# imatge-upc/rsis

Measured on AMD Instinct MI355X. Metric: training images/sec at 256x256, T=10, batch=32 per GPU, higher is better.
Workload: dtype f32

## Files before the change

### include/rsis_hip.h

```cpp
#ifndef RSIS_HIP_H
#define RSIS_HIP_H
#include <stddef.h>
#ifdef __cplusplus
extern "C" {
#endif

#define RSIS_ABI_VERSION 2

#define RSIS_DTYPE_F32 0
#define RSIS_DTYPE_BF16 1
#define RSIS_DTYPE_BF16_BLK 2
#define RSIS_DTYPE_F32_WINO 3

int rsis_version(void);
const char* rsis_error_string(int code);
int rsis_conv_uses_wino(int ks, int stride, int pad, int Cin, int Cout, int nseg, int lstm_hid);

int rsis_set_deterministic(int on);
int rsis_get_deterministic(void);

int rsis_conv_uses_bf16(int ks, int stride, int pad, int Cout);
long rsis_conv_packed_bytes_fwd(int dtype, int Cout, int ks, int stride, int pad, int nseg, const int* Cseg);
long rsis_conv_packed_bytes_dgrad(int dtype, int Cout, int ks, int stride, int pad, int c_count);
int rsis_conv_pack_fwd(const float* W, void* Wp, int Cout, int Ctot, int ks, int stride, int pad, int nseg, const int* Cseg,
                       const int* Coff, int lstm_hid, int dtype, void* stream);
int rsis_conv_pack_dgrad(const float* W, void* Wd, int Cout, int Ctot, int ks, int stride, int pad, int nseg, const int* Cseg,
                         const int* Coff, int lstm_hid, int dtype, void* stream);

int rsis_conv2d_fwd(const float* const* src, const int* Csrc, int nsrc, int B, int H, int W, const void* Wp, int Cout,
                    int ks, int stride, int pad, const float* bias, const float* addend, float* out, int Ho, int Wo,
                    int tile, int dtype, void* stream);
int rsis_conv2d_fwd_bn_eval(const float* const* src, const int* Csrc, int nsrc, int B, int H, int W, const void* Wp, int Cout,
                            int ks, int stride, int pad, const float* bias, const float* addend, const float* gamma, const float* beta,
                            const float* running_mean, const float* running_var, float eps, int relu, float* out, int Ho, int Wo,
                            int tile, int dtype, void* stream);

int rsis_conv2d_dgrad(const float* dy, int B, int Cout, int Hy, int Wy, const void* Wd, int Cin_packed, int ks, int stride,
                      int pad, float* const* dx, const int* Cdx, int ndst, int Hx, int Wx, const float* addend, int tile,
                      int dtype, void* stream);

int rsis_conv2d_wgrad(const float* dy, const float* x, float* dW, int B, int Cs, int H, int W, int Cout, int Ho, int Wo,
                      int ks, int stride, int pad, int Ctot, int c_off, int lstm_hid, int dtype, void* stream);

typedef struct rsis_wgrad_job {
  const float* dy;
  const float* x;
  float* dW;
  int B, Cs, H, W, Cout, Ho, Wo, ks, stride, pad, Ctot, c_off, lstm_hid, dtype;
} rsis_wgrad_job;
int rsis_conv2d_wgrad_batch(const rsis_wgrad_job* jobs, int njobs, void* stream);

int rsis_bias_grad(const float* dy, float* db, int B, int C, int HW, int lstm_hid, void* stream);

int rsis_convlstm_fwd(const float* const* src, const int* Csrc, int nsrc, int B, int H, int W, const void* Wp,
                      const float* bias_packed, const float* addend, const float* c_prev, float* h_out, float* c_out,
                      float* act_out, int hid, int ks, int pad, int tile, int dtype, void* stream);

typedef struct rsis_lstm_job {
  const float* src[3];
  int Csrc[3];
  int nsrc, B, H, W;
  const void* Wp;
// ... 266 lines not shown
```

### rsis_amd/_lib.py

```python
import ctypes
import os

import torch

_HERE = os.path.dirname(os.path.abspath(__file__))
LIB_PATH = os.environ.get("RSIS_HIP_LIB") or os.path.join(_HERE, "lib", "librsis_hip.so")

_vp, _i, _l, _f = ctypes.c_void_p, ctypes.c_int, ctypes.c_long, ctypes.c_float
_ip = ctypes.POINTER(ctypes.c_int)
_vpp = ctypes.POINTER(ctypes.c_void_p)

class PackJob(ctypes.Structure):
    _fields_ = [("W", ctypes.c_void_p), ("out", ctypes.c_void_p), ("dgrad", ctypes.c_int), ("dtype", ctypes.c_int), ("Cout", ctypes.c_int),
                ("Ctot", ctypes.c_int), ("ks", ctypes.c_int), ("stride", ctypes.c_int), ("pad", ctypes.c_int),
                ("nseg", ctypes.c_int), ("Cseg", ctypes.c_int * 3), ("Coff", ctypes.c_int * 3), ("lstm_hid", ctypes.c_int),
                ("imode", ctypes.c_int), ("ldw", ctypes.c_int), ("krows", ctypes.c_int), ("block_begin", ctypes.c_int)]


class WgradJob(ctypes.Structure):
    _fields_ = [("dy", ctypes.c_void_p), ("x", ctypes.c_void_p), ("dW", ctypes.c_void_p)] + \
               [(k, ctypes.c_int) for k in ("B", "Cs", "H", "W", "Cout", "Ho", "Wo", "ks", "stride", "pad", "Ctot", "c_off", "lstm_hid", "dtype")]


class LstmJob(ctypes.Structure):
# ... 30 lines not shown


class BlkLstmBwdJob(ctypes.Structure):
    _fields_ = [(k, ctypes.c_void_p) for k in ("dh", "dh2", "dc_next", "act", "c_prev", "c", "da", "dc_prev")] + \
               [(k, ctypes.c_int) for k in ("B", "hid", "HW")]


SIGNATURES = {
    "rsis_version": (_i, []),
    "rsis_error_string": (ctypes.c_char_p, [_i]),
    "rsis_set_deterministic": (_i, [_i]),
    "rsis_get_deterministic": (_i, []),
    "rsis_conv_uses_bf16": (_i, [_i, _i, _i, _i]),
    "rsis_conv_uses_wino": (_i, [_i, _i, _i, _i, _i, _i, _i]),
    "rsis_conv_packed_bytes_fwd": (_l, [_i, _i, _i, _i, _i, _i, _ip]),
    "rsis_conv_packed_bytes_dgrad": (_l, [_i, _i, _i, _i, _i, _i]),
    "rsis_conv_pack_fwd": (_i, [_vp, _vp, _i, _i, _i, _i, _i, _i, _ip, _ip, _i, _i, _vp]),
    "rsis_conv_pack_dgrad": (_i, [_vp, _vp, _i, _i, _i, _i, _i, _i, _ip, _ip, _i, _i, _vp]),
    "rsis_conv_pack_job_fill": (_i, [ctypes.POINTER(PackJob)]),
    "rsis_conv_pack_batch": (_i, [_vp, _i, _i, _vp]),
    "rsis_conv2d_fwd": (_i, [_vpp, _ip, _i, _i, _i, _i, _vp, _i, _i, _i, _i, _vp, _vp, _vp, _i, _i, _i, _i, _vp]),
    "rsis_conv2d_fwd_bn_eval": (_i, [_vpp, _ip, _i, _i, _i, _i, _vp, _i, _i, _i, _i, _vp, _vp, _vp, _vp, _vp, _vp, _f, _i, _vp, _i, _i, _i, _i, _vp]),
    "rsis_conv2d_dgrad": (_i, [_vp, _i, _i, _i, _i, _vp, _i, _i, _i, _i, _vpp, _ip, _i, _i, _i, _vp, _i, _i, _vp]),
    "rsis_conv2d_wgrad": (_i, [_vp, _vp, _vp, _i, _i, _i, _i, _i, _i, _i, _i, _i, _i, _i, _i, _i, _i, _vp]),
    "rsis_conv2d_wgrad_batch": (_i, [ctypes.POINTER(WgradJob), _i, _vp]),
    "rsis_affine_nearest": (_i, [_vp, _vp, _vp, _i, _i, _i, _i, _i, _vp]),
    "rsis_targets_work_ints": (_l, [_i]),
    "rsis_targets_from_maps": (_i, [_vp, _vp, _i, _i, _i, _i, _vp, _vp, _vp, _vp, _vp, _vp]),
    "rsis_instance_maps_work_ints": (_l, [_i]),
    "rsis_instance_maps": (_i, [_vp, _vp, _i, _i, _i, _i, _vp, _vp, _vp, _vp]),
    "rsis_palette_to_ids": (_i, [_vp, _l, _vp, _i, _vp, _vp]),
    "rsis_idmap_rle_encode": (_i, [_vp, _i, _i, _vp, _i, _vp, _i, _vp, _vp]),
    "rsis_conv_out_wgrad": (_i, [_vp, _vp, _vp, _vp, _i, _i, _i, _i, _vp]),
    "rsis_conv_out_seq_fwd": (_i, [_vp, _vp, _vp, _vp, _i, _i, _i, _i, _i, _vp]),
    "rsis_conv_out_seq_dgrad": (_i, [_vp, _vp, _vp, _i, _i, _i, _i, _i, _vp]),
    "rsis_conv_out_seq_wgrad": (_i, [_vp, _vp, _vp, _vp, _i, _i, _i, _i, _i, _vp]),
    "rsis_sum_leading": (_i, [_vp, _vp, _i, _l, _vp]),
    "rsis_bias_grad": (_i, [_vp, _vp, _i, _i, _i, _i, _vp]),
    "rsis_convlstm_fwd": (_i, [_vpp, _ip, _i, _i, _i, _i, _vp, _vp, _vp, _vp, _vp, _vp, _vp, _i, _i, _i, _i, _i, _vp]),
    "rsis_convlstm_fwd_batch": (_i, [ctypes.POINTER(LstmJob), _i, _vp]),
    "rsis_convlstm_bwd_gates": (_i, [_vp, _vp, _vp, _vp, _vp, _vp, _vp, _vp, _vp, _i, _i, _i, _vp]),
    "rsis_upsample_bilinear_ac_fwd": (_i, [_vp, _vp, _l, _i, _i, _i, _i, _vp]),
    "rsis_upsample_bilinear_ac_bwd": (_i, [_vp, _vp, _l, _i, _i, _i, _i, _vp]),
    "rsis_upsample_maxpool_bwd": (_i, [_vp, _vp, _vp, _vp, _l, _i, _i, _i, _i, _vp]),
    "rsis_global_maxpool_fwd": (_i, [_vp, _vp, _vp, _l, _i, _vp]),
    "rsis_global_maxpool_bwd": (_i, [_vp, _vp, _vp, _l, _i, _vp]),
# ... 129 lines not shown
```

### rsis_amd/csrc/api.hip

```cpp
#include "common.h"
#include "../../include/rsis_hip.h"
#include <stdlib.h>

int rsis_launch_conv_igemm(ConvArgs& a, int ks, bool dgrad, int epi, int force_tile, hipStream_t st);
int rsis_launch_conv_wgrad(WgradArgs& a, int ks, hipStream_t st);
int rsis_launch_conv3x3_direct(ConvArgs& a, int epi, int force_variant, hipStream_t st);
int rsis_launch_conv_wino(const float* x, const void* U, const float* bias, const float* addend, float* y, int B, int C, int Cout, int H, int W,
                          hipStream_t st, int precise);
int rsis_launch_conv_wino_group(int n, const float* const* x, const void* const* U, float* const* y, float* const* y1, const int* B, const int* C,
                                const int* Cout, const int* C0, const int* H, const int* W, hipStream_t st);
int rsis_launch_convlstm_direct_group(ConvArgs* jobs, int n, const int* force_variant, hipStream_t st);
int rsis_launch_conv3x3_direct_group_plain(ConvArgs* jobs, int n, const int* force_variant, hipStream_t st);
int rsis_l_lstm_bwd_group(const void* const*, const int*, int, hipStream_t);
int rsis_launch_conv_bf16(ConvArgs& a, int ks, int epi, int force_variant, hipStream_t st);
int rsis_launch_conv_blk(ConvArgs& a, int ks, int variant, hipStream_t st);
int rsis_l_blk_from_nchw(const float*, void*, int, int, int, hipStream_t);
int rsis_l_blk_to_nchw(const void*, float*, int, int, int, hipStream_t);
long rsis_l_blk_bn_scratch(int);
int rsis_l_blk_bn_fwd(const void*, const void*, void*, double*, const float*, const float*, float*, float*, float*, float*, int, int, int, float,
                      float, int, int, hipStream_t);
int rsis_l_blk_bn_bwd(const void*, const void*, const void*, double*, const float*, const float*, const float*, const float*, void*, void*,
                      float*, float*, int, int, int, int, int, hipStream_t);
int rsis_l_blk_subsample(const void*, void*, long, int, int, int, int, int, hipStream_t);
int rsis_l_blk_upscatter(const void*, void*, long, int, int, int, int, int, hipStream_t);
// ... 468 lines not shown
      const int nq = (Cout + RSIS_CK - 1) / RSIS_CK;
      const long px_tiles = (long)B * rsis_cdiv(Hx, 8) * rsis_cdiv(Wx, Wx <= 8 ? 8 : 16);
      if (splitk_ok && !addend && nq >= 32 && px_tiles * rsis_cdiv(ctot, 64) < 160) {
        for (int i = 0; i < ndst; ++i)
          if (rsis_zero_async(dx[i], sizeof(float) * (size_t)B * Cdx[i] * Hx * Wx, (hipStream_t)stream) != RSIS_OK) return RSIS_ERR_LAUNCH;
        a.ksplit = 0;
      }
    }
    return rsis_launch_conv3x3_direct(a, 0, direct_variant(tile), (hipStream_t)stream);
  }
  if (use_direct_s2(ks, stride, pad) && ndst == 1 && Cdx[0] == Cin_packed && Hy == (Hx + 1) / 2 && Wy == (Wx + 1) / 2) {
    a.Ho = Hy; a.Wo = Wy; a.oH = Hx; a.oW = Wx;
    return rsis_launch_conv3x3_direct(a, 2, direct_variant(tile), (hipStream_t)stream);
  }
  if (ks == 1 && pad == 0 && stride > 1) {
    for (int i = 0; i < ndst && !inplace; ++i)
      if (rsis_zero_async(dx[i], sizeof(float) * (size_t)B * Cdx[i] * Hx * Wx, (hipStream_t)stream) != RSIS_OK) return RSIS_ERR_LAUNCH;
    a.Ho = Hy; a.Wo = Wy; a.stride = 1; a.sshift = 0; a.ostride = stride;
    return rsis_launch_conv_igemm(a, ks, false, 0, tile, (hipStream_t)stream);
  }
  return rsis_launch_conv_igemm(a, ks, true, 0, tile, (hipStream_t)stream);
}

static int wgrad_route(WgradArgs& a, int ks, int lstm_hid, int dtype) {
  if (dtype == RSIS_DTYPE_BF16_BLK) {
    a.blk = 1;
    return rsis_wgrad_bf16_supported(a, ks) ? 1 : -1;
  }
  if (use_direct(ks, a.stride, a.pad) && a.Cout == 1 && lstm_hid == 0 && rsis_c1_supported(a.Cs) && a.H == a.Ho && a.W == a.Wo && a.W % 4 == 0)
    return 0;
  if (dtype == RSIS_DTYPE_BF16 && rsis_wgrad_bf16_supported(a, ks)) return 1;
  static const bool tiled_ok = !(getenv("RSIS_WGRAD_TILED") && getenv("RSIS_WGRAD_TILED")[0] == '0');
  if (tiled_ok && rsis_wgrad_tiled_supported(a, ks)) return 2;
  return 3;
}
static int wgrad_fill(WgradArgs& a, const float* dy, const float* x, float* dW, int B, int Cs, int H, int W, int Cout, int Ho, int Wo,
                      int ks, int stride, int pad, int Ctot, int c_off, int lstm_hid) {
  if (!dy || !x || !dW || c_off < 0 || c_off + Cs > Ctot) return RSIS_ERR_ARG;
  a = WgradArgs{};
  a.dy = dy; a.x = x; a.dw = dW; a.B = B; a.Cs = Cs; a.H = H; a.W = W; a.Ho = Ho; a.Wo = Wo; a.Cout = Cout;
  a.stride = stride; a.pad = pad; a.ldo = Ctot * ks * ks; a.n_off = c_off * ks * ks; a.interleave_hid = lstm_hid;
  return RSIS_OK;
}
static int wgrad_launch_one(WgradArgs& a, int route, int ks, hipStream_t st) {
  switch (route) {
    case 0: return rsis_l_c1_wgrad(a.dy, a.x, a.dw + a.n_off, nullptr, a.B, a.Cs, a.H, a.W, 1, st);
// ... 636 lines not shown
```

### rsis_amd/csrc/common.h

```cpp
#pragma once
#include <hip/hip_runtime.h>
#include <stdint.h>

#define RSIS_OK 0
#define RSIS_ERR_ARG 1
#define RSIS_ERR_LAUNCH 2
#define RSIS_ERR_UNSUPPORTED 3

#define RSIS_KPAD 32
#define RSIS_CK 8
#define RSIS_CKB3 16
#define RSIS_CKB1 64
#define RSIS_LDW_ALIGN 128
#define RSIS_MAX_SRC 3

typedef float f32x16 __attribute__((ext_vector_type(16)));
typedef float f32x4 __attribute__((ext_vector_type(4)));

static inline int rsis_check_launch() {
  hipError_t e = hipGetLastError();
  return e == hipSuccess ? RSIS_OK : RSIS_ERR_LAUNCH;
}

int rsis_zero_async(void* p, size_t bytes, hipStream_t st);
// ... 40 lines not shown
  int Ho, Wo;
  int stride, pad, sshift;
  const float* wp;
  int ldw;
  int Cout;
  const float* bias;
  const float* addend;
  const float* ep_gamma; const float* ep_beta; const float* ep_mean; const float* ep_var;
  float ep_eps;
  int ep_relu, ep_round;
  float* dst[RSIS_MAX_SRC];
  int Cd[RSIS_MAX_SRC];
  int ndst;
  int n_co_tiles, n_px_tiles;
  int ostride, oH, oW;
  int ksplit;
  int hid;
  const float* c_prev;
  float* h_out;
  float* c_out;
  float* act_out;
  unsigned long long* side_key;
  int precise;
};

__device__ __forceinline__ unsigned long long rsis_side_key(float v, int idx) {
  unsigned u = __float_as_uint(v);
  u = (u & 0x80000000u) ? ~u : (u | 0x80000000u);
  return ((unsigned long long)u << 32) | (unsigned)(0x7FFFFFFF - idx);
}
__device__ __forceinline__ float rsis_side_value(unsigned long long k) {
  unsigned u = (unsigned)(k >> 32);
  u = (u & 0x80000000u) ? (u & 0x7FFFFFFFu) : ~u;
  return __uint_as_float(u);
}
__device__ __forceinline__ int rsis_side_index(unsigned long long k) { return 0x7FFFFFFF - (int)(unsigned)(k & 0xFFFFFFFFull); }
__device__ __forceinline__ unsigned long long rsis_key_max32(unsigned long long k) {
#pragma unroll
  for (int o = 16; o > 0; o >>= 1) {
    const unsigned long long t = __shfl_xor(k, o, 64);
    k = t > k ? t : k;
  }
  return k;
}

#define RSIS_SIDE_CHECK_TILES 192
// ... 87 lines not shown
```

### rsis_amd/csrc/conv_igemm.hip

```cpp
#include "common.h"
#include <type_traits>

enum { EPI_PLAIN = 0, EPI_LSTM = 1, EPI_BN = 2 };
#ifndef RSIS_GEMM_NST_DEFAULT
#define RSIS_GEMM_NST_DEFAULT 2
#endif

typedef const float __attribute__((address_space(1)))* gcf_t;
typedef const char __attribute__((address_space(1)))* gcc_t;
typedef float __attribute__((address_space(1)))* gf_t;
typedef const f32x4 __attribute__((address_space(1)))* gcf4_t;

typedef __attribute__((address_space(3))) void* lds_vp_t;
template <int BM, int BN, int BK, int WGM, int WGN, int KS, bool DGRAD, int EPI, bool V4, int NST = 2>
__global__ __launch_bounds__(256) void conv_igemm_kernel(const ConvArgs p) {
#if __HIP_DEVICE_COMPILE__
  constexpr int TM = BM / WGM / 32, TN = BN / WGN / 32;
  constexpr int KK = KS * KS;
  constexpr int B_ROWS = 256 / BN;
  constexpr int B_LOADS = BK / B_ROWS;
  constexpr int A_F4 = BK * BM / 4;
  constexpr int A_LOADS = (A_F4 + 255) / 256;
  static_assert(WGM * WGN == 4, "4 waves per block");
  static_assert(BN == 64 || BN == 128 || BN == 256, "BN");
  static_assert(RSIS_KPAD % BK == 0, "BK must divide the packed K padding");
  static_assert(!V4 || (KS == 1 && !DGRAD), "V4 is the 1x1 GEMM path");
// ... 216 lines not shown
    if constexpr (V4) {
      __builtin_amdgcn_s_waitcnt(0x0F70);
    } else {
      if (more) RSIS_STORE_TILE(cur ^ 1)
    }
    __syncthreads();
  }
  }
#undef RSIS_LOAD_TILE
#undef RSIS_STORE_TILE
#undef RSIS_DMA_TILE

  if constexpr (EPI == EPI_BN) {
    if (tid < BM) {
      const int row = co_t * BM + tid;
      float sc = 0.f, sh = 0.f;
      if (row < p.Cout) rsis_bn_affine(rsis_bn_eval_rstd(p.ep_var[row], p.ep_eps), p.ep_gamma[row], p.ep_beta[row], p.ep_mean[row], sc, sh);
      lds[tid] = sc; lds[BM + tid] = sh;
    }
    __syncthreads();
  }
  const int co_base = co_t * BM + wm * TM * 32;
  const gcf_t bias = (gcf_t)p.bias, addend = (gcf_t)p.addend;
  if (EPI == EPI_PLAIN || EPI == EPI_BN) {
    const gf_t d0 = (gf_t)p.dst[0], d1 = (gf_t)p.dst[1], d2 = (gf_t)p.dst[2];
    const int Cd0 = p.Cd[0], Cd1 = p.Cd[1], Cd2 = p.Cd[2], Cout = p.Cout;
    const int e1 = Cd0, e2 = Cd0 + Cd1;
    const int ostride = p.ostride, oHW = p.oH * p.oW;
#pragma unroll
    for (int j = 0; j < TN; ++j) {
      const int opx = px_t * BN + wn * TN * 32 + j * 32 + l31;
      if (opx >= Npx) continue;
      const int ob = opx / HoWo;
      int osp = opx - ob * HoWo;
      if (ostride > 1) { const int oho = osp / Wo; osp = (oho * ostride) * p.oW + (osp - oho * Wo) * ostride; }
      if (p.ndst == 1 && (size_t)p.B * Cout * oHW * 4 < (1ull << 31)) {
        const unsigned span = (unsigned)((size_t)p.B * Cout * oHW * 4);
        const __amdgpu_buffer_rsrc_t ro = __builtin_amdgcn_make_buffer_rsrc((void*)p.dst[0], 0, span, 0x00020000);
        const __amdgpu_buffer_rsrc_t ra = __builtin_amdgcn_make_buffer_rsrc((void*)(addend ? p.addend : p.dst[0]), 0, span, 0x00020000);
        const unsigned rowb = (unsigned)oHW * 4u;
#pragma unroll
        for (int i = 0; i < TM; ++i) {
          const int row0 = co_base + i * 32 + 4 * hi;
          const unsigned vo = (unsigned)((ob * Cout + row0) * oHW + osp) * 4u;
          const int rows_left = Cout - row0;
          float av[16];
          if (addend) {
#pragma unroll
            for (int r = 0; r < 16; ++r) {
              const int k = (r & 3) + 8 * (r >> 2);
              av[r] = __builtin_bit_cast(float, __builtin_amdgcn_raw_buffer_load_b32(ra, k < rows_left ? vo + k * rowb : 0x7FFFFFF0u, 0, 0));
            }
          }
          if constexpr (EPI == EPI_BN) {
            const float* tab = lds + wm * TM * 32 + i * 32 + 4 * hi;
#pragma unroll
            for (int g = 0; g < 4; ++g) {
              const f32x4 s4 = *reinterpret_cast<const f32x4*>(tab + 8 * g), h4 = *reinterpret_cast<const f32x4*>(tab + BM + 8 * g);
#pragma unroll
              for (int kk = 0; kk < 4; ++kk) {
                const int r = 4 * g + kk, k = kk + 8 * g;
                float v = acc[i][j][r];
                if (bias) v += k < rows_left ? bias[row0 + k] : 0.f;
                v = rsis_bn_apply(v, s4[kk], h4[kk], addend ? av[r] : 0.f, p.ep_relu);
                __builtin_amdgcn_raw_buffer_store_b32(__builtin_bit_cast(unsigned, v), ro, k < rows_left ? vo + k * rowb : 0x7FFFFFF0u, 0, 0);
              }
            }
            continue;
          }
#pragma unroll
          for (int r = 0; r < 16; ++r) {
            const int k = (r & 3) + 8 * (r >> 2);
            float v = acc[i][j][r];
            if (bias) v += k < rows_left ? bias[row0 + k] : 0.f;
            if (addend) v += av[r];
            __builtin_amdgcn_raw_buffer_store_b32(__builtin_bit_cast(unsigned, v), ro, k < rows_left ? vo + k * rowb : 0x7FFFFFF0u, 0, 0);
          }
        }
        continue;
      }
#pragma unroll
      for (int i = 0; i < TM; ++i) {
        if (addend) {
          float av[16];
#pragma unroll
          for (int r = 0; r < 16; ++r) {
            const int co = co_base + i * 32 + (r & 3) + 8 * (r >> 2) + 4 * hi;
            av[r] = co < Cout ? addend[((size_t)ob * Cd0 + co) * oHW + osp] : 0.f;
          }
#pragma unroll
          for (int r = 0; r < 16; ++r) {
            const int co = co_base + i * 32 + (r & 3) + 8 * (r >> 2) + 4 * hi;
            if (co < Cout) d0[((size_t)ob * Cd0 + co) * oHW + osp] = acc[i][j][r] + av[r] + (bias ? bias[co] : 0.f);
          }
          continue;
        }
#pragma unroll
        for (int r = 0; r < 16; ++r) {
// ... 38 lines not shown
          const size_t sidx = ((size_t)ob * hid + jh) * HoWo + osp;
          const float cp = c_prev ? c_prev[sidx] : 0.f;
          const float c = gf * cp + gi * gg;
          const float h = go * tanhf(c);
          c_out[sidx] = c;
          h_out[sidx] = h;
          if (act_out) {
            act_out[gidx] = gi; act_out[gidx + HoWo] = gf;
            act_out[gidx + 2 * (size_t)HoWo] = go; act_out[gidx + 3 * (size_t)HoWo] = gg;
          }
        }
      }
    }
  }
#endif
}

template <int BM, int BN, int BK, int WGM, int WGN, int KS, bool DGRAD, int EPI>
static int launch_cfg(ConvArgs& a, hipStream_t st) {
  const long Npx = (long)a.B * a.Ho * a.Wo;
  a.n_co_tiles = rsis_cdiv(a.Cout, BM);
  a.n_px_tiles = rsis_cdiv(Npx, BN);
  const int grid = a.n_co_tiles * 8 * rsis_cdiv(a.n_px_tiles, 8);
  if constexpr (KS == 1 && !DGRAD && (EPI == EPI_PLAIN || EPI == EPI_BN)) {
    if (a.stride == 1 && a.pad == 0 && a.nsrc == 1 && (a.H * a.W) % 4 == 0 && a.C[0] % BK == 0 &&
        (long)a.B * a.C[0] * a.H * a.W * 4 < (1L << 31)) {
      if constexpr (BM == 64 && BN == 64 && BK == 32 && EPI == EPI_PLAIN) {
        static const int nst = getenv("RSIS_GEMM_NST") ? atoi(getenv("RSIS_GEMM_NST")) : RSIS_GEMM_NST_DEFAULT;
        if (nst == 3) { hipLaunchKernelGGL((conv_igemm_kernel<BM, BN, BK, WGM, WGN, KS, DGRAD, EPI, true, 3>), dim3(grid), dim3(256), 0, st, a); return rsis_check_launch(); }
        if (nst == 4) { hipLaunchKernelGGL((conv_igemm_kernel<BM, BN, BK, WGM, WGN, KS, DGRAD, EPI, true, 4>), dim3(grid), dim3(256), 0, st, a); return rsis_check_launch(); }
      }
      hipLaunchKernelGGL((conv_igemm_kernel<BM, BN, BK, WGM, WGN, KS, DGRAD, EPI, true>), dim3(grid), dim3(256), 0, st, a);
      return rsis_check_launch();
    }
  }
  hipLaunchKernelGGL((conv_igemm_kernel<BM, BN, BK, WGM, WGN, KS, DGRAD, EPI, false>), dim3(grid), dim3(256), 0, st, a);
  return rsis_check_launch();
}

template <int KS, bool DGRAD, int EPI>
static int launch_ks(ConvArgs& a, hipStream_t st, int force_tile) {
  const long Npx = (long)a.B * a.Ho * a.Wo;
  int tile = force_tile;
  if (tile <= 0) {
    if (a.Cout <= 32) tile = (Npx >= 256L * 256) ? 1 : 2;
    else if (KS == 1) tile = 5;
    else if (a.Cout <= 64) tile = 3;
// ... 8 lines not shown
    case 2: return launch_cfg<32, 128, 16, 1, 4, KS, DGRAD, EPI>(a, st);
    case 3: return launch_cfg<64, 128, 16, 2, 2, KS, DGRAD, EPI>(a, st);
    case 4: return launch_cfg<128, 128, 16, 2, 2, KS, DGRAD, EPI>(a, st);
    case 5: return launch_cfg<64, 64, 16, 2, 2, KS, DGRAD, EPI>(a, st);
    case 6: return launch_cfg<128, 64, 16, 2, 2, KS, DGRAD, EPI>(a, st);
    case 11: return launch_cfg<32, 256, 32, 1, 4, KS, DGRAD, EPI>(a, st);
    case 12: return launch_cfg<32, 128, 32, 1, 4, KS, DGRAD, EPI>(a, st);
    case 13: return launch_cfg<64, 128, 32, 2, 2, KS, DGRAD, EPI>(a, st);
    case 14: return launch_cfg<128, 128, 32, 2, 2, KS, DGRAD, EPI>(a, st);
    case 15: return launch_cfg<64, 64, 32, 2, 2, KS, DGRAD, EPI>(a, st);
    case 16: return launch_cfg<128, 64, 32, 2, 2, KS, DGRAD, EPI>(a, st);
    default: return RSIS_ERR_ARG;
  }
}

int rsis_launch_conv_igemm(ConvArgs& a, int ks, bool dgrad, int epi, int force_tile, hipStream_t st) {
  if (a.nsrc < 0 || a.nsrc > RSIS_MAX_SRC) return RSIS_ERR_ARG;
  if (epi == EPI_LSTM) {
    if (dgrad) return RSIS_ERR_UNSUPPORTED;
    if (ks == 3) return launch_ks<3, false, EPI_LSTM>(a, st, force_tile);
    if (ks == 1) return launch_ks<1, false, EPI_LSTM>(a, st, force_tile);
    return RSIS_ERR_UNSUPPORTED;
  }
  if (a.ep_gamma) {
    if (dgrad || epi != EPI_PLAIN || a.ndst != 1 || a.Cout <= 32 || a.Cout % 4 != 0 || (size_t)a.B * a.Cout * a.oH * a.oW * 4 >= (1ull << 31))
      return RSIS_ERR_UNSUPPORTED;
    if (ks == 1) return launch_cfg<64, 64, 32, 2, 2, 1, false, EPI_BN>(a, st);
    if (ks == 7 && a.Cout <= 64) return launch_cfg<64, 128, 32, 2, 2, 7, false, EPI_BN>(a, st);
    return RSIS_ERR_UNSUPPORTED;
  }
  if (!dgrad) {
    if (ks == 1) return launch_ks<1, false, EPI_PLAIN>(a, st, force_tile);
    if (ks == 3) return launch_ks<3, false, EPI_PLAIN>(a, st, force_tile);
    if (ks == 7) return launch_ks<7, false, EPI_PLAIN>(a, st, force_tile);
  } else {
    if (ks == 1 && a.stride == 1 && a.pad == 0) return launch_ks<1, false, EPI_PLAIN>(a, st, force_tile);
    if (ks == 1) return launch_ks<1, true, EPI_PLAIN>(a, st, force_tile);
    if (ks == 3) return launch_ks<3, true, EPI_PLAIN>(a, st, force_tile);
    if (ks == 7) return launch_ks<7, true, EPI_PLAIN>(a, st, force_tile);
  }
  return RSIS_ERR_UNSUPPORTED;
}
```

### rsis_amd/ops.py

```python
import ctypes
import os
import weakref

import torch

from . import _lib
from ._lib import check, int_array, lib, ptr, ptr_array, require_cuda_f32, stream

_WEIGHT_EPOCH = [0]


FORCE_TILE = [0]


DIRECT_GRAD = [False]


def _direct_target(param):
    g = param.grad if DIRECT_GRAD[0] and param is not None else None
    return g if (g is not None and g.is_contiguous() and g.dtype == torch.float32 and g.is_cuda) else None


DTYPE_F32, DTYPE_BF16 = 0, 1
DTYPE_F32_WINO = 3
# ... 21 lines not shown
        return d
    return DTYPE_F32_WINO if (rule == "all" or (cin == cout and cin in rule)) else d

DTYPES = {"fp32": DTYPE_F32, "f32": DTYPE_F32, "float32": DTYPE_F32, "bf16": DTYPE_BF16, "bfloat16": DTYPE_BF16}


def set_dtype(module, dtype):
    d = DTYPES[dtype] if isinstance(dtype, str) else int(dtype)
    for m in module.modules():
        if hasattr(m, "_set_rsis_dtype"):
            m._set_rsis_dtype(d)
    return module


def set_deterministic(on=True):
    return bool(lib().rsis_set_deterministic(1 if on else 0))


def is_deterministic():
    return bool(lib().rsis_get_deterministic())


SUBSAMPLE_1X1 = [os.environ.get("RSIS_SUBSAMPLE_1X1", "1") != "0"]
_PACKS = weakref.WeakSet()
_BATCH = {"sig": None, "jobs": None, "n": 0, "blocks": 0}


def repack_all():
    L = lib()
    todo = []
    for p in list(_PACKS):
        w = p._refs[0]() if p._refs is not None else None
        if w is None or not w.is_cuda:
            continue
        b = p._refs[1]() if p._refs[1] is not None else None
        if p.wp is not None and p._key_f is not None:
            todo.append((p, w, b, p.wp, 0))
        if p.wd is not None and p._key_d is not None:
            todo.append((p, w, b, p.wd, 1))
    if not todo:
        return
    sig = tuple((id(p), w.data_ptr(), out.data_ptr(), d) for p, w, _b, out, d in todo)
    if _BATCH["sig"] != sig:
        jobs = (_lib.PackJob * len(todo))()
        blocks = 0
        for i, (p, w, _b, out, d) in enumerate(todo):
# ... 94 lines not shown
            L = lib()
            Cout, Ctot = w.shape[0], w.shape[1]
            nseg, segs, offs = self._seg_args()
            n = L.rsis_conv_packed_bytes_dgrad(self.dtype, Cout, self.ks, self.stride, self.pad, self.cin) // 4
            if self.wd is None or self.wd.numel() != n:
                self.wd = torch.zeros(n, dtype=torch.float32, device=w.device)
            check(L.rsis_conv_pack_dgrad(ptr(w.detach()), ptr(self.wd), Cout, Ctot, self.ks, self.stride, self.pad, nseg, segs, offs,
                                         self.lstm_hid, self.dtype, stream()), "rsis_conv_pack_dgrad")
            self._key_d = key
            if self._refs is None:
                self._refs = (weakref.ref(w), None)
            _PACKS.add(self)
        return self.wd


def _contig(t):
    return t if t.is_contiguous() else t.contiguous()


def _conv_out_size(n, ks, stride, pad):
    return (n + 2 * pad - ks) // stride + 1


def _dgrad_all(L, dy, wd, cin_packed, ks, stride, pad, srcs, Hx, Wx, addend=None, inplace=False, dtype=DTYPE_F32):
    B, Cout, Hy, Wy = dy.shape
    shapes = [tuple(s.shape) if torch.is_tensor(s) else tuple(s) for s in srcs]
    dxs = [addend] if inplace else [torch.empty(sh, dtype=torch.float32, device=dy.device) for sh in shapes]
    check(L.rsis_conv2d_dgrad(ptr(dy), B, Cout, Hy, Wy, ptr(wd), cin_packed, ks, stride, pad, ptr_array(dxs),
                              int_array([sh[1] for sh in shapes]), len(shapes), Hx, Wx, ptr(addend), FORCE_TILE[0], dtype, stream()),
          "rsis_conv2d_dgrad")
    return dxs


class GradSlot(object):

    def __init__(self):
        self.grad = None
        self.done = False

    def reset(self):
        self.grad, self.done = None, False

    def take(self):
        g, self.grad = self.grad, None
        self.done = True
        return g

    def park(self, g):
        if self.done or self.grad is not None or g is None:
            return False
        self.grad = g
        return True


class _GradTapFn(torch.autograd.Function):
    @staticmethod
    def forward(ctx, x, slot):
        ctx.slot = slot
        return x.view_as(x)

    @staticmethod
    def backward(ctx, g):
        if g is not None and ctx.slot.park(g if g.is_contiguous() else g.contiguous()):
            return None, None
        return g, None


def grad_tap(x, slot):
    if slot is None or not (torch.is_grad_enabled() and x.requires_grad):
        return x
    return _GradTapFn.apply(x, slot)


WGRAD_DEFER = [False]
# ... 43 lines not shown
        require_cuda_f32(weight, bias, *srcs)
        L = lib()
        B, _, H, W = srcs[0].shape
        Cout, ks = weight.shape[0], weight.shape[2]
        Ho, Wo = _conv_out_size(H, ks, stride, pad), _conv_out_size(W, ks, stride, pad)
        if pack.stride != stride or pack.pad != pad:
            raise _lib.RsisHipError("PackedConv was built for stride %d pad %d, used with %d/%d" % (pack.stride, pack.pad, stride, pad))
        wp = pack.fwd(weight)
        out = torch.empty((B, Cout, Ho, Wo), dtype=torch.float32, device=weight.device)
        ctx.in_shape = None
        if ks == 1 and stride > 1 and pad == 0 and nsrc == 1 and (SUBSAMPLE_1X1[0] or pack.dtype == DTYPE_BF16):
            ctx.in_shape = tuple(srcs[0].shape)
            sub = torch.empty((B, srcs[0].shape[1], Ho, Wo), dtype=torch.float32, device=weight.device)
            check(L.rsis_subsample2d(ptr(srcs[0]), ptr(sub), B * srcs[0].shape[1], H, W, stride, stream()), "rsis_subsample2d")
            srcs = [sub]
            H, W, stride_k = Ho, Wo, 1
        else:
            stride_k = stride
        tile = FORCE_TILE[0] + (100 if pack.training_call else 0)
        check(L.rsis_conv2d_fwd(ptr_array(srcs), int_array([s.shape[1] for s in srcs]), nsrc, B, H, W, ptr(wp), Cout, ks, stride_k,
                                pad, ptr(bias.detach() if bias is not None else None), None, ptr(out), Ho, Wo, tile, pack.dtype, stream()),
              "rsis_conv2d_fwd")
        ctx.pack, ctx.stride, ctx.pad, ctx.nsrc = pack, stride, pad, nsrc
        ctx.has_bias = bias is not None
        ctx.wparam, ctx.bparam = weight, bias
        ctx.save_for_backward(weight, *srcs)
        return out

    @staticmethod
    def backward(ctx, dy):
        weight = ctx.saved_tensors[0]
        srcs = list(ctx.saved_tensors[1:])
        dy = _contig(dy)
        L = lib()
        ks = weight.shape[2]
        nsrc = ctx.nsrc
        grads = [None] * (nsrc + 2)
        take, park = ctx.slot if isinstance(ctx.slot, tuple) else (ctx.slot, None)
        addend = take.take() if take is not None else None
        sub = ctx.in_shape is not None
        in_shapes = [ctx.in_shape] if sub else [tuple(t.shape) for t in srcs]
        if any(ctx.needs_input_grad[5:5 + nsrc]):
            wd = ctx.pack.dgrad(weight)
            inplace, extra = False, None
            if addend is not None:
                if nsrc != 1 or tuple(addend.shape) != in_shapes[0]:
                    raise _lib.RsisHipError("GradSlot: the parked gradient does not belong to this conv's input")
                if ctx.stride != 1:
                    if ks == 1 and ctx.pad == 0 and addend.is_contiguous():
                        inplace = True
                    else:
                        extra, addend = addend, None
            dxs = _dgrad_all(L, dy, wd, ctx.pack.cin, ks, ctx.stride, ctx.pad, in_shapes, in_shapes[0][2], in_shapes[0][3], addend,
                             inplace, dtype=ctx.pack.dtype)
            if extra is not None:
                dxs[0].add_(extra)
            for i in range(nsrc):
                if ctx.needs_input_grad[5 + i]:
                    grads[i] = dxs[i]
            if park is not None and nsrc == 1 and grads[0] is not None and park.park(grads[0]):
                grads[0] = None
        want_w = ctx.needs_input_grad[5 + nsrc]
        want_b = ctx.has_bias and ctx.needs_input_grad[6 + nsrc]
        if (want_w and want_b and weight.shape[0] == 1 and ks == 3 and ctx.stride == 1 and ctx.pad == 1 and nsrc == 1 and
                weight.shape[1] in (4, 8, 16) and srcs[0].shape[3] % 4 == 0):
            tw, tb = _direct_target(ctx.wparam), _direct_target(ctx.bparam)
            dW = tw if tw is not None else torch.zeros_like(weight)
            db = tb if tb is not None else torch.zeros(1, dtype=torch.float32, device=dy.device)
            x0 = srcs[0]
            check(L.rsis_conv_out_wgrad(ptr(dy), ptr(x0), ptr(dW), ptr(db), x0.shape[0], x0.shape[1], x0.shape[2], x0.shape[3], stream()),
                  "rsis_conv_out_wgrad")
            grads[nsrc] = None if tw is not None else dW
            grads[nsrc + 1] = None if tb is not None else db
            return (None, None, None, None, None) + tuple(grads)
        if want_w:
            tgt = _direct_target(ctx.wparam)
            dW = _wgrad_all(L, dy, srcs, tuple(weight.shape), ks, 1 if sub else ctx.stride, ctx.pad, 0, out=tgt, dtype=ctx.pack.dtype)
# ... 225 lines not shown
        x, y, gamma, mean, rstd = ctx.saved_tensors
        dy = _contig(dy)
        B, C, H, W = x.shape
        if not ctx.train:
            stats = torch.empty(2 * C, dtype=torch.float64, device=dy.device)
            dx = torch.empty_like(x)
            need_dres = ctx.has_res and ctx.relu
            dres = torch.empty_like(x) if need_dres else None
            dgamma = torch.empty(C, dtype=torch.float32, device=dy.device)
            dbeta = torch.empty_like(dgamma)
            fn, name = (lib().rsis_bn_bwd_eval_mask, "rsis_bn_bwd_eval_mask") if ctx.masked else (lib().rsis_bn_bwd_eval, "rsis_bn_bwd_eval")
            check(fn(ptr(dy), ptr(x), ptr(y), ptr(mean), ptr(rstd), ptr(gamma.detach()), ptr(stats), ptr(dx), ptr(dres),
                     ptr(dgamma), ptr(dbeta), B, C, H * W, float(ctx.eps), int(ctx.relu), stream()), name)
            if ctx.has_res and not need_dres:
                dres = dy
            return dx, dres, dgamma, dbeta, None, None, None, None, None, None, None, None, None
        flags = int(ctx.relu)
        if ctx.arena is not None:
            stats, flags = ctx.arena[1], flags | 2
        else:
            stats = torch.empty(2 * C, dtype=torch.float64, device=dy.device)
        dx = torch.empty_like(x)
        need_dres = ctx.has_res and ctx.relu
        dres = torch.empty_like(x) if need_dres else None
        tg, tb = _direct_target(ctx.gparam), _direct_target(ctx.bparam)
        direct = tg is not None and tb is not None
        if direct:
            dgamma, dbeta, flags = tg, tb, flags | 4
        else:
            dgamma = torch.empty(C, dtype=torch.float32, device=dy.device)
            dbeta = torch.empty_like(dgamma)
        fn, name = (lib().rsis_bn_bwd_mask, "rsis_bn_bwd_mask") if ctx.masked else (lib().rsis_bn_bwd, "rsis_bn_bwd")
        check(fn(ptr(dy), ptr(x), ptr(y), ptr(mean), ptr(rstd), ptr(gamma.detach()), ptr(stats), ptr(dx), ptr(dres),
                 ptr(dgamma), ptr(dbeta), B, C, H * W, flags, stream()), name)
        if ctx.has_res and not need_dres:
            dres = dy
        if direct:
            dgamma = dbeta = None
        if ctx.res_slot is not None and ctx.res_slot.park(dres):
            dres = None
        return dx, dres, dgamma, dbeta, None, None, None, None, None, None, None, None, None


def batchnorm(x, gamma, beta, running_mean, running_var, train, relu=False, res=None, eps=1e-5, momentum=0.1, arena=None,
              res_slot=None):
    want_grad = torch.is_grad_enabled() and any(t is not None and t.requires_grad for t in (x, res, gamma, beta))
    return _BatchNormFn.apply(x, res, gamma, beta, running_mean, running_var, bool(train), bool(relu), eps, momentum, arena,
# ... 404 lines not shown
```

Before: 967.5.

## Fuse masked residual gradient into 1x1 dgrad epilogue instead of materializing dres

When a masked BN+ReLU backward has a residual branch feeding a 1x1 conv, the BN backward now parks dy plus the packed ReLU mask bytes in the gradient slot instead of writing a separate dres tensor. The 1x1 dgrad kernel gets a new masked epilogue that loads the mask bits and adds dy only where the ReLU was active. This removes one full-size tensor write and its later read in the residual path, at the cost of an extra byte-load per output group, and the new path is pinned to a single 64x64x32 tile config.

Result: no change. 972.7, median of 6 (+0.5%).

```diff
diff --git a/include/rsis_hip.h b/include/rsis_hip.h
--- a/include/rsis_hip.h
+++ b/include/rsis_hip.h
@@ -38,6 +38,11 @@
 int rsis_conv2d_dgrad(const float* dy, int B, int Cout, int Hy, int Wy, const void* Wd, int Cin_packed, int ks, int stride,
                       int pad, float* const* dx, const int* Cdx, int ndst, int Hx, int Wx, const float* addend, int tile,
                       int dtype, void* stream);
+
+int rsis_conv_dgrad_maskadd_ok(int B, int ks, int stride, int pad, int ndst, int Cdx, int Hx, int Wx, int dtype);
+int rsis_conv2d_dgrad_maskadd(const float* dy, int B, int Cout, int Hy, int Wy, const void* Wd, int Cin_packed, int ks, int stride,
+                              int pad, float* const* dx, const int* Cdx, int ndst, int Hx, int Wx, const float* addend,
+                              const unsigned char* addend_mask, int tile, int dtype, void* stream);
 
 int rsis_conv2d_wgrad(const float* dy, const float* x, float* dW, int B, int Cs, int H, int W, int Cout, int Ho, int Wo,
                       int ks, int stride, int pad, int Ctot, int c_off, int lstm_hid, int dtype, void* stream);
diff --git a/rsis_amd/_lib.py b/rsis_amd/_lib.py
--- a/rsis_amd/_lib.py
+++ b/rsis_amd/_lib.py
@@ -76,6 +76,8 @@
     "rsis_conv2d_fwd": (_i, [_vpp, _ip, _i, _i, _i, _i, _vp, _i, _i, _i, _i, _vp, _vp, _vp, _i, _i, _i, _i, _vp]),
     "rsis_conv2d_fwd_bn_eval": (_i, [_vpp, _ip, _i, _i, _i, _i, _vp, _i, _i, _i, _i, _vp, _vp, _vp, _vp, _vp, _vp, _f, _i, _vp, _i, _i, _i, _i, _vp]),
     "rsis_conv2d_dgrad": (_i, [_vp, _i, _i, _i, _i, _vp, _i, _i, _i, _i, _vpp, _ip, _i, _i, _i, _vp, _i, _i, _vp]),
+    "rsis_conv_dgrad_maskadd_ok": (_i, [_i, _i, _i, _i, _i, _i, _i, _i, _i]),
+    "rsis_conv2d_dgrad_maskadd": (_i, [_vp, _i, _i, _i, _i, _vp, _i, _i, _i, _i, _vpp, _ip, _i, _i, _i, _vp, _vp, _i, _i, _vp]),
     "rsis_conv2d_wgrad": (_i, [_vp, _vp, _vp, _i, _i, _i, _i, _i, _i, _i, _i, _i, _i, _i, _i, _i, _i, _vp]),
     "rsis_conv2d_wgrad_batch": (_i, [ctypes.POINTER(WgradJob), _i, _vp]),
     "rsis_affine_nearest": (_i, [_vp, _vp, _vp, _i, _i, _i, _i, _i, _vp]),
diff --git a/rsis_amd/csrc/api.hip b/rsis_amd/csrc/api.hip
--- a/rsis_amd/csrc/api.hip
+++ b/rsis_amd/csrc/api.hip
@@ -514,6 +514,31 @@
   return rsis_launch_conv_igemm(a, ks, true, 0, tile, (hipStream_t)stream);
 }
 
+int rsis_conv_dgrad_maskadd_ok(int B, int ks, int stride, int pad, int ndst, int Cdx, int Hx, int Wx, int dtype) {
+  return dtype == RSIS_DTYPE_F32 && ks == 1 && stride == 1 && pad == 0 && ndst == 1 && B >= 1 && Cdx >= 1 && Hx >= 1 && Wx >= 1 &&
+         ((long)Hx * Wx) % 4 == 0 && (size_t)B * Cdx * Hx * Wx * 4 < (1ull << 31);
+}
+
+int rsis_conv2d_dgrad_maskadd(const float* dy, int B, int Cout, int Hy, int Wy, const void* Wd, int Cin_packed, int ks, int stride,
+                              int pad, float* const* dx, const int* Cdx, int ndst, int Hx, int Wx, const float* addend,
+                              const unsigned char* addend_mask, int tile, int dtype, void* stream) {
+  if (!dy || !Wd || !dx || !Cdx || !addend || !addend_mask || ndst < 1 || ndst > RSIS_MAX_SRC) return RSIS_ERR_ARG;
+  if (!dx[0] || Cdx[0] < 1) return RSIS_ERR_ARG;
+  if (!rsis_conv_dgrad_maskadd_ok(B, ks, stride, pad, ndst, Cdx[0], Hx, Wx, dtype)) return RSIS_ERR_UNSUPPORTED;
+  if (Hx != Hy || Wx != Wy || Cdx[0] > Cin_packed) return RSIS_ERR_ARG;
+  ConvArgs a = {};
+  const float* srcs[1] = {dy};
+  const int cs[1] = {Cout};
+  const int rc = fill_sources(a, srcs, cs, 1, ks);
+  if (rc) return rc;
+  a.dst[0] = dx[0]; a.Cd[0] = Cdx[0]; a.ndst = 1;
+  a.B = B; a.H = Hy; a.W = Wy; a.Ho = Hx; a.Wo = Wx; a.stride = 1; a.pad = 0; a.sshift = 0;
+  a.ostride = 1; a.oH = Hx; a.oW = Wx; a.ksplit = 1;
+  a.wp = (const float*)Wd; a.ldw = rsis_roundup(Cin_packed, RSIS_LDW_ALIGN); a.Cout = Cdx[0]; a.bias = nullptr;
+  a.addend = addend; a.addend_mask = addend_mask;
+  return rsis_launch_conv_igemm(a, 1, true, 3 , tile, (hipStream_t)stream);
+}
+
 static int wgrad_route(WgradArgs& a, int ks, int lstm_hid, int dtype) {
   if (dtype == RSIS_DTYPE_BF16_BLK) {
     a.blk = 1;
diff --git a/rsis_amd/csrc/common.h b/rsis_amd/csrc/common.h
--- a/rsis_amd/csrc/common.h
+++ b/rsis_amd/csrc/common.h
@@ -86,6 +86,7 @@
   float* act_out;
   unsigned long long* side_key;
   int precise;
+  const unsigned char* addend_mask;
 };
 
 __device__ __forceinline__ unsigned long long rsis_side_key(float v, int idx) {
diff --git a/rsis_amd/csrc/conv_igemm.hip b/rsis_amd/csrc/conv_igemm.hip
--- a/rsis_amd/csrc/conv_igemm.hip
+++ b/rsis_amd/csrc/conv_igemm.hip
@@ -1,7 +1,7 @@
 #include "common.h"
 #include <type_traits>
 
-enum { EPI_PLAIN = 0, EPI_LSTM = 1, EPI_BN = 2 };
+enum { EPI_PLAIN = 0, EPI_LSTM = 1, EPI_BN = 2, EPI_MASK = 3 };
 #ifndef RSIS_GEMM_NST_DEFAULT
 #define RSIS_GEMM_NST_DEFAULT 2
 #endif
@@ -264,7 +264,7 @@
   }
   const int co_base = co_t * BM + wm * TM * 32;
   const gcf_t bias = (gcf_t)p.bias, addend = (gcf_t)p.addend;
-  if (EPI == EPI_PLAIN || EPI == EPI_BN) {
+  if (EPI == EPI_PLAIN || EPI == EPI_BN || EPI == EPI_MASK) {
     const gf_t d0 = (gf_t)p.dst[0], d1 = (gf_t)p.dst[1], d2 = (gf_t)p.dst[2];
     const int Cd0 = p.Cd[0], Cd1 = p.Cd[1], Cd2 = p.Cd[2], Cout = p.Cout;
     const int e1 = Cd0, e2 = Cd0 + Cd1;
@@ -276,7 +276,7 @@
       const int ob = opx / HoWo;
       int osp = opx - ob * HoWo;
       if (ostride > 1) { const int oho = osp / Wo; osp = (oho * ostride) * p.oW + (osp - oho * Wo) * ostride; }
-      if (p.ndst == 1 && (size_t)p.B * Cout * oHW * 4 < (1ull << 31)) {
+      if (EPI == EPI_MASK || (p.ndst == 1 && (size_t)p.B * Cout * oHW * 4 < (1ull << 31))) {
         const unsigned span = (unsigned)((size_t)p.B * Cout * oHW * 4);
         const __amdgpu_buffer_rsrc_t ro = __builtin_amdgcn_make_buffer_rsrc((void*)p.dst[0], 0, span, 0x00020000);
         const __amdgpu_buffer_rsrc_t ra = __builtin_amdgcn_make_buffer_rsrc((void*)(addend ? p.addend : p.dst[0]), 0, span, 0x00020000);
@@ -287,7 +287,16 @@
           const unsigned vo = (unsigned)((ob * Cout + row0) * oHW + osp) * 4u;
           const int rows_left = Cout - row0;
           float av[16];
-          if (addend) {
+          [[maybe_unused]] unsigned mb[16];
+          if constexpr (EPI == EPI_MASK) {
+            const __amdgpu_buffer_rsrc_t rm = __builtin_amdgcn_make_buffer_rsrc((void*)p.addend_mask, 0, span >> 4, 0x00020000);
+#pragma unroll
+            for (int r = 0; r < 16; ++r) {
+              const int k = (r & 3) + 8 * (r >> 2);
+              mb[r] = __builtin_amdgcn_raw_buffer_load_b8(rm, k < rows_left ? (vo >> 4) + k * (rowb >> 4) : 0x7FFFFFF0u, 0, 0);
+            }
+          }
+          if (EPI == EPI_MASK || addend) {
 #pragma unroll
             for (int r = 0; r < 16; ++r) {
               const int k = (r & 3) + 8 * (r >> 2);
@@ -315,7 +324,8 @@
             const int k = (r & 3) + 8 * (r >> 2);
             float v = acc[i][j][r];
             if (bias) v += k < rows_left ? bias[row0 + k] : 0.f;
-            if (addend) v += av[r];
+            if constexpr (EPI == EPI_MASK) v += ((mb[r] >> (osp & 3)) & 1u) ? av[r] : 0.f;
+            else if (addend) v += av[r];
             __builtin_amdgcn_raw_buffer_store_b32(__builtin_bit_cast(unsigned, v), ro, k < rows_left ? vo + k * rowb : 0x7FFFFFF0u, 0, 0);
           }
         }
@@ -400,7 +410,7 @@
   a.n_co_tiles = rsis_cdiv(a.Cout, BM);
   a.n_px_tiles = rsis_cdiv(Npx, BN);
   const int grid = a.n_co_tiles * 8 * rsis_cdiv(a.n_px_tiles, 8);
-  if constexpr (KS == 1 && !DGRAD && (EPI == EPI_PLAIN || EPI == EPI_BN)) {
+  if constexpr (KS == 1 && !DGRAD && (EPI == EPI_PLAIN || EPI == EPI_BN || EPI == EPI_MASK)) {
     if (a.stride == 1 && a.pad == 0 && a.nsrc == 1 && (a.H * a.W) % 4 == 0 && a.C[0] % BK == 0 &&
         (long)a.B * a.C[0] * a.H * a.W * 4 < (1L << 31)) {
       if constexpr (BM == 64 && BN == 64 && BK == 32 && EPI == EPI_PLAIN) {
@@ -455,6 +465,12 @@
     if (ks == 1) return launch_ks<1, false, EPI_LSTM>(a, st, force_tile);
     return RSIS_ERR_UNSUPPORTED;
   }
+  if (epi == EPI_MASK) {
+    if (!dgrad || ks != 1 || a.stride != 1 || a.pad != 0 || a.ndst != 1 || !a.addend || !a.addend_mask || a.ep_gamma || a.ostride != 1 ||
+        (a.oH * a.oW) % 4 != 0 || (size_t)a.B * a.Cout * a.oH * a.oW * 4 >= (1ull << 31))
+      return RSIS_ERR_UNSUPPORTED;
+    return launch_cfg<64, 64, 32, 2, 2, 1, false, EPI_MASK>(a, st);
+  }
   if (a.ep_gamma) {
     if (dgrad || epi != EPI_PLAIN || a.ndst != 1 || a.Cout <= 32 || a.Cout % 4 != 0 || (size_t)a.B * a.Cout * a.oH * a.oW * 4 >= (1ull << 31))
       return RSIS_ERR_UNSUPPORTED;
diff --git a/rsis_amd/ops.py b/rsis_amd/ops.py
--- a/rsis_amd/ops.py
+++ b/rsis_amd/ops.py
@@ -67,6 +67,7 @@
 
 
 SUBSAMPLE_1X1 = [os.environ.get("RSIS_SUBSAMPLE_1X1", "1") != "0"]
+MASKED_RES = [os.environ.get("RSIS_MASKED_RES", "1") != "0"]
 _PACKS = weakref.WeakSet()
 _BATCH = {"sig": None, "jobs": None, "n": 0, "blocks": 0}
 
@@ -207,10 +208,21 @@
     return (n + 2 * pad - ks) // stride + 1
 
 
-def _dgrad_all(L, dy, wd, cin_packed, ks, stride, pad, srcs, Hx, Wx, addend=None, inplace=False, dtype=DTYPE_F32):
+def _maskadd_ok(L, B, ks, stride, pad, shapes, dtype):
+    return bool(L.rsis_conv_dgrad_maskadd_ok(B, ks, stride, pad, len(shapes), shapes[0][1], shapes[0][2], shapes[0][3], dtype))
+
+
+def _dgrad_all(L, dy, wd, cin_packed, ks, stride, pad, srcs, Hx, Wx, addend=None, inplace=False, dtype=DTYPE_F32, addend_mask=None):
     B, Cout, Hy, Wy = dy.shape
     shapes = [tuple(s.shape) if torch.is_tensor(s) else tuple(s) for s in srcs]
     dxs = [addend] if inplace else [torch.empty(sh, dtype=torch.float32, device=dy.device) for sh in shapes]
+    if addend_mask is not None:
+        if addend is None or inplace or not addend.is_contiguous() or addend_mask.numel() * 4 != addend.numel():
+            raise _lib.RsisHipError("GradSlot: the parked mask bytes do not belong to the parked gradient")
+        check(L.rsis_conv2d_dgrad_maskadd(ptr(dy), B, Cout, Hy, Wy, ptr(wd), cin_packed, ks, stride, pad, ptr_array(dxs),
+                                          int_array([sh[1] for sh in shapes]), len(shapes), Hx, Wx, ptr(addend), ptr(addend_mask),
+                                          FORCE_TILE[0], dtype, stream()), "rsis_conv2d_dgrad_maskadd")
+        return dxs
     check(L.rsis_conv2d_dgrad(ptr(dy), B, Cout, Hy, Wy, ptr(wd), cin_packed, ks, stride, pad, ptr_array(dxs),
                               int_array([sh[1] for sh in shapes]), len(shapes), Hx, Wx, ptr(addend), FORCE_TILE[0], dtype, stream()),
           "rsis_conv2d_dgrad")
@@ -221,20 +233,32 @@
 
     def __init__(self):
         self.grad = None
+        self.mask = None
         self.done = False
+        self.takes_mask = False
 
     def reset(self):
-        self.grad, self.done = None, False
+        self.grad, self.mask, self.done, self.takes_mask = None, None, False, False
 
     def take(self):
         g, self.grad = self.grad, None
         self.done = True
         return g
 
+    def take_mask(self):
+        m, self.mask = self.mask, None
+        return m
+
     def park(self, g):
         if self.done or self.grad is not None or g is None:
             return False
         self.grad = g
+        return True
+
+    def park_masked(self, g, mask):
+        if not self.takes_mask or mask is None or not self.park(g):
+            return False
+        self.mask = mask
         return True
 
 
@@ -324,6 +348,9 @@
                                 pad, ptr(bias.detach() if bias is not None else None), None, ptr(out), Ho, Wo, tile, pack.dtype, stream()),
               "rsis_conv2d_fwd")
         ctx.pack, ctx.stride, ctx.pad, ctx.nsrc = pack, stride, pad, nsrc
+        take = slot[0] if isinstance(slot, tuple) else slot
+        if take is not None:
+            take.takes_mask = MASKED_RES[0] and nsrc == 1 and _maskadd_ok(L, B, ks, stride, pad, [tuple(srcs[0].shape)], pack.dtype)
         ctx.has_bias = bias is not None
         ctx.wparam, ctx.bparam = weight, bias
         ctx.save_for_backward(weight, *srcs)
@@ -340,6 +367,7 @@
         grads = [None] * (nsrc + 2)
         take, park = ctx.slot if isinstance(ctx.slot, tuple) else (ctx.slot, None)
         addend = take.take() if take is not None else None
+        addend_mask = take.take_mask() if take is not None else None
         sub = ctx.in_shape is not None
         in_shapes = [ctx.in_shape] if sub else [tuple(t.shape) for t in srcs]
         if any(ctx.needs_input_grad[5:5 + nsrc]):
@@ -354,7 +382,7 @@
                     else:
                         extra, addend = addend, None
             dxs = _dgrad_all(L, dy, wd, ctx.pack.cin, ks, ctx.stride, ctx.pad, in_shapes, in_shapes[0][2], in_shapes[0][3], addend,
-                             inplace, dtype=ctx.pack.dtype)
+                             inplace, dtype=ctx.pack.dtype, addend_mask=addend_mask)
             if extra is not None:
                 dxs[0].add_(extra)
             for i in range(nsrc):
@@ -626,7 +654,9 @@
             stats = torch.empty(2 * C, dtype=torch.float64, device=dy.device)
         dx = torch.empty_like(x)
         need_dres = ctx.has_res and ctx.relu
-        dres = torch.empty_like(x) if need_dres else None
+        handed = (need_dres and ctx.masked and MASKED_RES[0] and ctx.res_slot is not None and dy.shape == x.shape and
+                  ctx.res_slot.park_masked(dy, y))
+        dres = torch.empty_like(x) if need_dres and not handed else None
         tg, tb = _direct_target(ctx.gparam), _direct_target(ctx.bparam)
         direct = tg is not None and tb is not None
         if direct:
```
